# jennyzhang0215/DGL-KGAT

Hardware: AMD Instinct MI355X
Metric: propagation-layer edges/sec on amazon-book CKG; achieved HBM GB/s vs peak (higher is better)
Workload: dtype f32; 1 GPU; amazon-book-shaped CKG N=159251 E=3663302 R=41, 3 layers, embed_dim=64, fp32; partition=none, setup_steps=1, full=False

## Files before the change

### dgl-kgat_amd/_lib.py

```python
import ctypes as C
import hashlib
import os
import subprocess

_HERE = os.path.dirname(os.path.abspath(__file__))
CSRC = os.path.join(_HERE, "csrc")
SO_PATH = os.path.join(_HERE, "libkgat_hip.so")
SOURCES = {
    "kgat_graph.hip": [],
    "kgat_permute.hip": [],
    "kgat_spmm.hip": [],
    "kgat_spmm_max.hip": [],
    "kgat_spmm_kmax.hip": [],
    "kgat_spmm_bi.hip": ["-mllvm", "-amdgpu-mfma-vgpr-form=1"],
    "kgat_softmax.hip": [],
    "kgat_att.hip": [],
    "kgat_att_persistent.hip": ["-mllvm", "-amdgpu-mfma-vgpr-form=1"],
    "kgat_dense.hip": ["-mllvm", "-amdgpu-mfma-vgpr-form=1"],
    "kgat_transr.hip": [],
    "kgat_transr_rank.hip": ["-mllvm", "-amdgpu-mfma-vgpr-form=1"],
    "kgat_eval.hip": [],
    "kgat_eval_topk.hip": ["-mllvm", "-amdgpu-mfma-vgpr-form=1"],
    "kgat_optim.hip": [],
    "kgat_bpr.hip": [],
# ... 69 lines not shown
    "kgat_transr_loss_grad_f32": (_i32, [_i64, _i32, _i32, _i32, _i64, _p, _p, _p, _p, _p, _p, _p, C.c_float, _p, _p,
                                         _p, _p, _p, _sz, _p]),
    "kgat_transr_forward_f32": (_i32, [_i64, _i32, _i32, _i32, _i64, _p, _p, _p, _p, _p, _p, _p, C.c_float, _p, _p, _sz, _p]),
    "kgat_transr_backward_f32": (_i32, [_i64, _i32, _i32, _i32, _i64, _p, _p, _p, _p, _p, _p, _p, _p, _p, _sz, _p]),
    "kgat_bi_interaction_f32": (_i32, [_i64, _i32, _i32, _p, _p, C.c_float, _p, _p, _i64, _p]),
    "kgat_spmm_tile_edges": (_i32, [_i64, _i32]),
    "kgat_l2_normalize_rows_f32": (_i32, [_i64, _i32, _p, _p, _i64, _p]),
    "kgat_readout_concat_f32": (_i32, [_i64, _i32, _p, _p, _p, _p, _i64, _p]),
    "kgat_sddmm_dot_f32": (_i32, [_i64, _i32, _p, _p, _p, _p, _p, _p]),
    "kgat_gather_probe_f32": (_i32, [_i64, _i32, _p, _p, _p, _p]),
    "kgat_gather_f32": (_i32, [_i64, _p, _p, _p, _p]),
    "kgat_gather_i32": (_i32, [_i64, _p, _p, _p, _p]),
    "kgat_permute_tile": (_i32, []),
    "kgat_permute_supported": (_i32, [_i64]),
    "kgat_permute_f32": (_i32, [_i64, _p, _p, _p, _p, _p, _p, _p]),
    "kgat_eval_supported": (_i32, [_i32, _i32]),
    "kgat_eval_items_elems": (_i64, [_i64, _i32]),
    "kgat_eval_items_kmajor_f32": (_i32, [_i64, _i32, _p, _i64, _p, _p, _p]),
    "kgat_eval_workspace_bytes": (_sz, [_i64, _i64, _i32, _i32]),
    "kgat_bpr_workspace_bytes": (_sz, [_i64, _i32]),
    "kgat_bpr_loss_f32": (_i32, [_i64, _i32, _p, _i64, _i64, _p, _p, _p, C.c_float, _p, _p, _p, _sz, _p]),
    "kgat_bpr_grad_f32": (_i32, [_i64, _i32, _p, _i64, _i64, _p, _p, _p, _p, C.c_float, _p, _p, _p, _sz, _p]),
    "kgat_transr_sorted_bytes": (_sz, [_i64, _i32]),
    "kgat_transr_presort_f32": (_i32, [_i64, _i32, _i64, _i64, _p, _p, _p, _p, _p, _sz, _p]),
    "kgat_transr_step_workspace_bytes": (_sz, [_i64, _i32, _i32, _i32]),
    "kgat_transr_adam_step_f32": (_i32, [_i64, _i32, _i32, _i32, _i64, _p, _p, _p, _p, _p, _p, _p, _p, _p, _p, _p,
                                         C.c_double, C.c_double, C.c_double, C.c_double, C.c_float, _p, _p, C.c_uint64,
                                         _p, _sz, _p]),
    "kgat_adam_max_tensors": (_i32, []),
    "kgat_adam_step_f32": (_i32, [_i32, _p, _p, _p, _p, _p, _p, C.c_double, C.c_double, C.c_double, C.c_double, _i32, _p]),
# ... 200 lines not shown
```

### dgl-kgat_amd/csrc/kgat_permute.hip

```cpp
#include "kgat_common.h"

#ifndef KGAT_PERMUTE_TILE
#define KGAT_PERMUTE_TILE 16384
#endif

namespace {

using namespace kgat;

constexpr int kPermTile = KGAT_PERMUTE_TILE;
constexpr int kPermThreads = 1024;
constexpr int kPermMinRun = 16;
static_assert(kPermTile % (kPermThreads * 8) == 0 && kPermTile <= 65536, "tile: whole 8-item rounds, 16-bit slots");

typedef uint32_t u32x4 __attribute__((ext_vector_type(4)));

__device__ __forceinline__ void scatter_to_lds(const uint32_t* __restrict__ val, const uint16_t* __restrict__ slot, int cnt,
                                               uint32_t* lds) {
  constexpr int kRounds = kPermTile / (kPermThreads * 8);
  u32x4 lo[kRounds], hi[kRounds], s[kRounds];
#pragma unroll
  for (int r = 0; r < kRounds; ++r) {
    const int i = (r * kPermThreads + (int)threadIdx.x) * 8;
    if (i + 8 <= cnt) {
// ... 44 lines not shown
  __shared__ __attribute__((aligned(16))) uint32_t lds[kPermTile];
  constexpr int kRounds = kPermTile / (kPermThreads * 4);
  const int64_t base = (int64_t)blockIdx.x * kPermTile;
  const int cnt = (int)(n - base < kPermTile ? n - base : kPermTile);
  scatter_to_lds(tmp + base, slot_b + base, cnt, lds);
  __syncthreads();
#pragma unroll
  for (int r = 0; r < kRounds; ++r) {
    const int i = (r * kPermThreads + (int)threadIdx.x) * 4;
    if (i + 4 <= cnt) {
      __builtin_nontemporal_store(*reinterpret_cast<const u32x4*>(lds + i), reinterpret_cast<u32x4*>(out + base + i));
    } else {
      for (int k = i; k < cnt; ++k) out[base + k] = lds[k];
    }
  }
}

}

extern "C" {

int kgat_permute_tile(void) { return kPermTile; }

int kgat_permute_supported(int64_t n) {
  return n >= 0 && n * kPermMinRun <= (int64_t)kPermTile * kPermTile ? 1 : 0;
}

int kgat_permute_f32(int64_t n, const uint16_t* slot_a, const int32_t* dst_a, const uint16_t* slot_b, const float* in,
                     float* out, float* tmp, kgat_stream_t stream) {
  KGAT_CHECK_ARG(n >= 0, "permute: negative size");
// ... 23 lines not shown
```

### dgl-kgat_amd/csrc/kgat_softmax.hip

```cpp
#include <math.h>

#include "kgat_common.h"

#define SM_LD_LOGIT(p) (*(p))
#define SM_LD_MAP(p) __builtin_nontemporal_load(p)
namespace kgat {

constexpr float kFixScale = 1099511627776.0f;
constexpr float kFixInv = 1.0f / 1099511627776.0f;

__global__ void softmax_init_kernel(int64_t n, float* __restrict__ M,
                                    unsigned long long* __restrict__ Z) {
  const int64_t i = (int64_t)blockIdx.x * blockDim.x + threadIdx.x;
  if (i < n) {
    M[i] = -INFINITY;
    Z[i] = 0ull;
  }
}

__device__ __forceinline__ void atomic_max_f32(float* addr, float v) {
  if (v == 0.f) v = 0.f;
  if (v >= 0.f) atomicMax(reinterpret_cast<int*>(addr), __float_as_int(v));
  else atomicMin(reinterpret_cast<unsigned int*>(addr), __float_as_uint(v));
}
// ... 99 lines not shown
    e[k] = valid ? (eid ? eid[p[k]] : (int32_t)p[k]) : 0;
  }
#pragma unroll
  for (int k = 0; k < kItems; ++k) {
    s[k] = r[k] >= 0 ? (IN_CSR ? logits[p[k]] : logits[e[k]]) : 0.f;
    m[k] = r[k] >= 0 ? M[r[k]] : 0.f;
    z[k] = r[k] >= 0 ? Z[r[k]] : 1ull;
  }
#pragma unroll
  for (int k = 0; k < kItems; ++k) {
    if (r[k] < 0) continue;
    const float a = expf(s[k] - m[k]) / ((float)z[k] * kFixInv);
    if (out_csr) out_csr[p[k]] = a;
    if (out) out[e[k]] = a;
  }
}

constexpr int kSmMaxEPL = 16;
constexpr int64_t kSmSmallEdges = 8 << 20;
template <int EPL> struct SmGeom {
  static constexpr int EPW = kWave * EPL;
};
constexpr float kSmNegBig = -3.0e38f;

struct __attribute__((aligned(16))) SmCarry {
  int32_t row;
  int32_t count;
  float m, s;
  int32_t head;
  int32_t last;
  int32_t pad0, pad1;
};

__device__ __forceinline__ float sm_exp(float x) {
  x = fmaxf(x, -128.0f);
  const float t = x * 1.44269504088896341f;
  const float lo = fmaf(x, 1.44269504088896341f, -t) + x * 1.92596299112661746e-8f;
  return __builtin_amdgcn_exp2f(t) * fmaf(lo, 0.693147180559945309f, 1.0f);
}

__device__ __forceinline__ void sm_combine(float& m, float& s, float m2, float s2) {
  const bool keep = m >= m2;
  const float e = sm_exp(keep ? m2 - m : m - m2);
  const float big = keep ? s : s2, small = keep ? s2 : s;
  s = fmaf(small, e, big);
  m = keep ? m : m2;
}

__device__ __forceinline__ int64_t sm_wave_index() {
  return (int64_t)blockIdx.x * (256 / kWave) + __builtin_amdgcn_readfirstlane((int)(threadIdx.x / kWave));
}

template <int CTRL, int ROW_MASK>
__device__ __forceinline__ float sm_dpp(float old, float src) {
  return __int_as_float(__builtin_amdgcn_update_dpp(__float_as_int(old), __float_as_int(src), CTRL, ROW_MASK, 0xf, false));
}
template <int CTRL>
__device__ __forceinline__ int32_t sm_dpp_i(int32_t old, int32_t src) {
  return __builtin_amdgcn_update_dpp(old, src, CTRL, 0xf, 0xf, false);
}

// ... 226 lines not shown

template <bool IN_CSR, int kSmEPL>
__global__ __launch_bounds__(256) void softmax_local_kernel(
    int64_t e0, int64_t e1, int aligned, const int32_t* __restrict__ indptr, const int32_t* __restrict__ row_of,
    const int32_t* __restrict__ eid, const float* __restrict__ logits, float* __restrict__ out,
    float* __restrict__ out_csr, SmCarry* __restrict__ carry) {
  constexpr int kSmEPW = SmGeom<kSmEPL>::EPW;
  const int64_t w = sm_wave_index();
  const int64_t base = e0 + w * kSmEPW;
  if (base >= e1) return;
  const int64_t end = base + kSmEPW < e1 ? base + kSmEPW : e1;
  if (aligned && end - base == kSmEPW)
    sm_sweep<IN_CSR, kSmEPL, true>(e0, e1, w, base, end, indptr, row_of, eid, logits, out, out_csr, carry);
  else
    sm_sweep<IN_CSR, kSmEPL, false>(e0, e1, w, base, end, indptr, row_of, eid, logits, out, out_csr, carry);
}

__device__ __forceinline__ void sm_chain_total(const SmCarry* __restrict__ carry, int32_t head, int32_t last,
                                               int lane, float& M, float& S) {
  const SmCarry h = carry[2 * (int64_t)head + 1];
  float m = h.m, s = h.s;
  for (int64_t j0 = (int64_t)head + 1; j0 <= last; j0 += kWave) {
    const int64_t j = j0 + lane;
    float pm = kSmNegBig, ps = 0.f;
    if (j <= last) {
      const SmCarry f = carry[2 * j];
      pm = f.m; ps = f.s;
    }
#pragma unroll
    for (int d = 1; d < kWave; d <<= 1) {
      const float m2 = __shfl_down(pm, d, kWave), s2 = __shfl_down(ps, d, kWave);
      if ((lane & (2 * d - 1)) == 0) sm_combine(pm, ps, m2, s2);
    }
    pm = __shfl(pm, 0, kWave); ps = __shfl(ps, 0, kWave);
    sm_combine(m, s, pm, ps);
  }
  M = m; S = s;
}

__device__ __forceinline__ void sm_rescale_span(int64_t lo, int64_t hi, int lane, float f,
                                                const int32_t* __restrict__ eid, float* __restrict__ out,
                                                float* __restrict__ out_csr) {
  constexpr int U = 8;
  for (int64_t p0 = lo; p0 < hi; p0 += U * kWave) {
    int64_t e[U];
    float x[U];
#pragma unroll
    for (int u = 0; u < U; ++u) {
      const int64_t p = p0 + u * kWave + lane;
      const int64_t pc = p < hi ? p : hi - 1;
      e[u] = out ? (int64_t)eid[pc] : pc;
    }
// ... 86 lines not shown
#pragma unroll
  for (int off = kWave / 2; off > 0; off >>= 1) acc += __shfl_xor(acc, off, kWave);
  for (int32_t p = beg + lane; p < end; p += kWave) {
    const int32_t e = HAS_EID ? eid[p] : p;
    gs[e] = a[e] * g[e] - a[e] * acc;
  }
}

}

using namespace kgat;

template <bool IN_CSR, int EPL>
static void launch_softmax_sweep(int64_t e_begin, int64_t e_end, const int32_t* indptr, const int32_t* row_of,
                                 const int32_t* eid, const float* logits, float* out, float* out_csr, SmCarry* carry,
                                 hipStream_t st) {
  const int64_t n_waves = (e_end - e_begin + SmGeom<EPL>::EPW - 1) / SmGeom<EPL>::EPW;
  const unsigned blocks = (unsigned)((n_waves + 3) / 4);
  const uintptr_t bits = (uintptr_t)row_of | (uintptr_t)eid | (uintptr_t)out_csr | (IN_CSR ? (uintptr_t)logits : 0);
  const int aligned = (bits % 16 == 0 && e_begin % 4 == 0) ? 1 : 0;
  hipLaunchKernelGGL((softmax_local_kernel<IN_CSR, EPL>), dim3(blocks), dim3(256), 0, st, e_begin, e_end, aligned, indptr,
                     row_of, eid, logits, out, out_csr, carry);
  hipLaunchKernelGGL((softmax_cut_rows_kernel<EPL>), dim3(blocks), dim3(256), 0, st, e_begin, e_end, eid, out, out_csr,
                     (const SmCarry*)carry);
}

extern "C" {

size_t kgat_edge_softmax_workspace_bytes(int64_t n_nodes, int64_t n_edges) {
  (void)n_nodes;
  constexpr int kMinEPW = SmGeom<8>::EPW;
  const size_t n_waves = (size_t)((n_edges > 0 ? n_edges : 0) + kMinEPW - 1) / kMinEPW;
  return align_up((2 * n_waves + 2) * sizeof(SmCarry), 256);
}

int kgat_edge_softmax_f32(int64_t n_nodes, int64_t e_begin, int64_t e_end, const int32_t* indptr,
                          const int32_t* row_of, const int32_t* eid, const float* logits,
// ... 11 lines not shown
    set_error("edge_softmax: workspace too small");
    return KGAT_E_WORKSPACE;
  }
  hipStream_t st = as_stream(stream);
  SmCarry* carry = static_cast<SmCarry*>(workspace);
  const bool small = ne < kSmSmallEdges;
  if (logits_in_csr_order) {
    if (small) launch_softmax_sweep<true, 8>(e_begin, e_end, indptr, row_of, eid, logits, out, out_csr, carry, st);
    else launch_softmax_sweep<true, 16>(e_begin, e_end, indptr, row_of, eid, logits, out, out_csr, carry, st);
  } else {
    if (small) launch_softmax_sweep<false, 8>(e_begin, e_end, indptr, row_of, eid, logits, out, out_csr, carry, st);
    else launch_softmax_sweep<false, 16>(e_begin, e_end, indptr, row_of, eid, logits, out, out_csr, carry, st);
  }
  KGAT_CHECK_LAUNCH("edge_softmax");
  return KGAT_OK;
}

size_t kgat_edge_softmax_3pass_workspace_bytes(int64_t n_nodes) {
  const size_t n = (size_t)(n_nodes > 0 ? n_nodes : 1);
  return align_up(n * sizeof(float), 256) + align_up(n * sizeof(unsigned long long), 256);
}

int kgat_edge_softmax_3pass_f32(int64_t n_nodes, int64_t e_begin, int64_t e_end,
                                const int32_t* row_of, const int32_t* eid, const float* logits,
                                int logits_in_csr_order, float* out, float* out_csr, void* workspace,
                                size_t workspace_bytes, kgat_stream_t stream) {
  KGAT_CHECK_ARG(n_nodes >= 0 && e_begin >= 0 && e_end >= e_begin && e_end < INT32_MAX,
                 "edge_softmax_3pass: bad size");
  if (e_end == e_begin) return KGAT_OK;
  KGAT_CHECK_ARG(row_of && logits && workspace, "edge_softmax_3pass: null pointer");
// ... 56 lines not shown
```

### dgl-kgat_amd/graph.py

```python
from collections import namedtuple
from collections.abc import MutableMapping

import os

import numpy as np
import torch

from . import ops
from .options import options
from .function import BuiltinMessage, BuiltinReduce
from .lazy import LazyEdgeWeights, pending_csr_weights

ALL = "__ALL__"


class DGLError(Exception):
    """Same role as dgl.DGLError: misuse of the graph API."""


def _as_id_array(x, name):
    if isinstance(x, torch.Tensor):
        x = x.detach().cpu().numpy()
    x = np.asarray(x)
    if x.ndim == 0:
# ... 174 lines not shown
            et32 = etype.to(device=dev, dtype=torch.int32).contiguous()
            rel_ptr, idx = ops.group_by_relation(ops.gather(csr.eid, et32), int(n_rel))
            dst_g = ops.gather(idx, csr.row_of)
            gid, gptr, g_node, n_groups = ops.head_groups(rel_ptr, dst_g)
            hit = ((etype._version, int(n_rel)),
                   RelGroups(rel_ptr, ops.gather(idx, csr.eid), ops.gather(idx, csr.col), dst_g, idx,
                             gid, gptr, g_node, n_groups, {}), etype)
            c["rel_groups"] = hit
        return hit[1]

    def permuted(self, name, src_of, values, out=None):
        planned = (values.dtype == torch.float32 and ops.permute_supported(src_of.numel())
                   and values.data_ptr() % 16 == 0 and (out is None or out.data_ptr() % 16 == 0))
        if not planned:
            return ops.gather(src_of, values, out=out)
        c = self._cache(values.device)
        plan = c.get(("permute_plan", name))
        if plan is None or plan[0] is not src_of:
            plan = c[("permute_plan", name)] = (src_of, ops.permute_plan(src_of))
        tmp = c.get("permute_tmp")
        if tmp is None or tmp.numel() != src_of.numel():
            tmp = c["permute_tmp"] = torch.empty(src_of.numel(), dtype=torch.float32, device=values.device)
        return ops.permute(plan[1], values, out=out, tmp=tmp)

    def weight_in_csr_order(self, w_flat):
        c = self._cache(w_flat.device)
        key = (w_flat.data_ptr(), w_flat._version, w_flat.numel())
        hit = c.get("w_csr")
        if hit is None or hit[0] != key:
            hit = (key, self.permuted("csr_eid", self.csr(w_flat.device).eid, w_flat), w_flat)
            c["w_csr"] = hit
        return hit[1]

    def weight_in_rev_order(self, w_flat):
        c = self._cache(w_flat.device)
        key = (w_flat.data_ptr(), w_flat._version, w_flat.numel())
        hit = c.get("w_rev")
        if hit is None or hit[0] != key:
# ... 432 lines not shown
                                 ent_c, W_c, rel_c, pos_g=groups.pos_g, algo=one_algo)[1]

        forms = {"fused": (fused, "grouped"), "folded": (lambda: two_launch(True), "csr"),
                 "split": (lambda: two_launch(False), "csr"), "one": (one, "csr")}
        form, one_algo = options.att_form if algo == "auto" else algo, "auto"
        if form in ("auto", "race"):
            race_run = (lambda f: forms[f][0]()) if form == "race" else None
            form = groups.g_tab.get(("form", d, k))
            if form is None:
                form = groups.g_tab[("form", d, k)] = self._pick_attention_form(groups, n_rel, d, k, race_run)
        elif form not in forms:
            form, one_algo = "one", form
        run, order = forms[form]
        logits = run()
        st.last_att_form = (form, groups.n_groups)
        _, a_csr = ops.edge_softmax(csr.indptr, csr.row_of, _gpos_csr(groups) if order == "grouped" else csr.eid, logits,
                                    in_csr_order=order == "csr", want_out=False, want_csr=True)
        from . import lazy as lazy_mod
        if lazy is None:
            lazy = lazy_mod.enabled()
        elif lazy:
            lazy_mod._guard_legacy_to_dlpack()
        a = torch.empty((st.n_edges, 1), dtype=torch.float32, device=dev)
        a_flat = a.view(-1)

        def fill():
            st.permuted("csr_pos", st.csr_pos(dev), a_csr, out=a_flat)
            st.remember_weight(a_flat, a_csr)
        if not lazy:
            fill()
            return a
        return LazyEdgeWeights(a, fill, st, a_csr)
```

### dgl-kgat_amd/ops.py

```python
from collections import namedtuple

import torch

from . import _lib
from ._lib import KGATLibraryError, check

SPMM_MUL_SELF = 1
SPMM_DEFER_FINISH = 2
SPMM_ALGO = {"auto": 0, "merge": 1, "rows": 2, "generic": 3, "merge1": 4}
ATT_ALGO = {"auto": 0, "mfma": 1, "generic": 2, "mfma_chunk": 3}


def _stream(t):
    return torch.cuda.current_stream(t.device).cuda_stream


class KernelTimer:
    active = None

    def __init__(self):
        self.records = []

    def __enter__(self):
        KernelTimer.active = self
# ... 516 lines not shown
    out_csr = torch.empty_like(logits) if want_csr else None
    with _timed("edge_softmax", (e1 - e0,)):
        if three_pass:
            ws = _workspace(lib.kgat_edge_softmax_3pass_workspace_bytes(n_nodes), logits.device)
            check(lib.kgat_edge_softmax_3pass_f32(n_nodes, e0, e1, _ptr(row_of), _ptr(eid), _ptr(logits),
                                                  1 if in_csr_order else 0, _ptr(out), _ptr(out_csr), _ptr(ws),
                                                  ws.numel(), _stream(logits)), "kgat_edge_softmax_3pass_f32")
        else:
            ws = _workspace(lib.kgat_edge_softmax_workspace_bytes(n_nodes, e1 - e0), logits.device)
            check(lib.kgat_edge_softmax_f32(n_nodes, e0, e1, _ptr(indptr), _ptr(row_of), _ptr(eid), _ptr(logits),
                                            1 if in_csr_order else 0, _ptr(out), _ptr(out_csr), _ptr(ws),
                                            ws.numel(), _stream(logits)), "kgat_edge_softmax_f32")
    return out, out_csr


def edge_softmax_bwd(indptr, eid, a, grad_a, row_range=None):
    a = _need(a, torch.float32, "a")
    grad_a = _need(grad_a, torch.float32, "grad_a", a.shape)
    indptr = _need(indptr, torch.int32, "indptr")
    if eid is not None:
        eid = _need(eid, torch.int32, "eid", a.shape)
    row0, n_rows = (0, indptr.numel() - 1) if row_range is None else row_range
    out = torch.zeros_like(a)
    if a.numel() == 0:
        return out
    check(_lib.load().kgat_edge_softmax_bwd_f32(n_rows, row0, _ptr(indptr), _ptr(eid), _ptr(a),
                                                _ptr(grad_a), _ptr(out), _stream(a)),
          "kgat_edge_softmax_bwd_f32")
    return out

# ... 582 lines not shown
def sddmm_dot(src, dst, X, G):
    X = _need(X, torch.float32, "X")
    G = _need(G, torch.float32, "grad_out")
    src = _need(src, torch.int32, "src")
    dst = _need(dst, torch.int32, "dst", src.shape)
    if X.shape[1] != G.shape[1]:
        raise ValueError("feature widths differ")
    out = torch.empty(src.numel(), dtype=torch.float32, device=X.device)
    check(_lib.load().kgat_sddmm_dot_f32(src.numel(), X.shape[1], _ptr(src), _ptr(dst), _ptr(X), _ptr(G),
                                         _ptr(out), _stream(X)), "kgat_sddmm_dot_f32")
    return out


__all__ = ["csr_from_coo", "group_by_relation", "invert_permutation", "row_order_by_degree", "gather",
           "permute_tile", "permute_supported", "permute_plan_arrays", "permute_plan", "permute", "PermutePlan",
           "att_score", "att_score_split", "att_score_split_supported", "att_score_folded_supported", "att_score_fused", "att_pack_records", "att_score_fused_supported", "fold_tiles", "fold_tile_cost", "bi_interaction_train", "add3_rows", "bi_interaction_bwd_pre", "bi_interaction_bwd_input", "bi_interaction_bwd_input_supported", "bi_interaction_bwd_weight", "sum_partials", "mul2", "dropout_keep_mask", "transr_loss_grad", "transr_supported", "transr_presort", "transr_adam_step", "TransRAdamState", "head_groups", "edge_softmax", "edge_softmax_bwd", "spmm", "spmm_workspace", "sddmm_dot",
           "bi_interaction", "bi_interaction_supported", "l2_normalize_rows", "readout_concat",
           "FORMS", "aggregator", "aggregator_supported", "aggregator_bwd_supported", "aggregator_train",
           "aggregator_bwd_input", "aggregator_bwd_weight",
           "KGATLibraryError"]


def eval_supported(F, K):
    return bool(_lib.load().kgat_eval_supported(int(F), int(K)))


def eval_recall_ndcg(emb, user_ids, item_ids, train_ptr, train_items, test_ptr, test_items, K, want_topk=False):
    if emb.dtype != torch.float32 or not emb.is_cuda or emb.dim() != 2 or emb.stride(1) != 1:
        raise KGATLibraryError("eval_recall_ndcg: `emb` must be a float32 HIP matrix with unit column stride")
    F, stride = emb.shape[1], emb.stride(0)
    user_ids = _need(user_ids, torch.int32, "user_ids")
# ... 304 lines not shown
```

### dgl-kgat_amd/options.py

```python
import contextlib
import os


def _flag(name, default):
    v = os.environ.get(name)
    return default if v is None else v not in ("", "0")


class Options:
    __slots__ = ("att_f32_products", "att_form", "fold_tile_cost", "fuse_bi", "gnn_defer_finish", "lazy_edge_weights",
                 "eager_edge_weights", "partition_row_weight", "force_collectives", "exchange", "exchange_chunks")

    def __init__(self):
        self.load()

    def load(self):
        e = os.environ
        self.att_f32_products = _flag("KGAT_ATT_F32_PRODUCTS", False)
        self.att_form = e.get("KGAT_ATT_FORM", "auto")
        cost = e.get("KGAT_FOLD_TILE_COST")
        self.fold_tile_cost = tuple(int(x) for x in cost.split(",")) if cost else None
        self.fuse_bi = _flag("KGAT_FUSE_BI", False)
        self.gnn_defer_finish = _flag("KGAT_GNN_DEFER_FINISH", True)
        self.lazy_edge_weights = _flag("KGAT_LAZY_EDGE_WEIGHTS", False)
        self.eager_edge_weights = bool(e.get("KGAT_EAGER_EDGE_WEIGHTS"))
        rw = e.get("KGAT_PARTITION_ROW_WEIGHT")
        self.partition_row_weight = int(rw) if rw else None
        self.force_collectives = _flag("KGAT_FORCE_COLLECTIVES", False)
        self.exchange = e.get("KGAT_EXCHANGE", "allreduce")
        self.exchange_chunks = int(e.get("KGAT_EXCHANGE_CHUNKS", "1"))


options = Options()


def reload():
    options.load()
    return options


# ... 11 lines not shown
```

### include/kgat_hip.h

```cpp
#ifndef KGAT_HIP_H_
#define KGAT_HIP_H_

#include <stddef.h>
#include <stdint.h>

#ifdef __cplusplus
extern "C" {
#endif

#define KGAT_ABI_VERSION 16

enum {
  KGAT_OK = 0,
  KGAT_E_BADARG = -1,
  KGAT_E_UNSUPPORTED = -2,
  KGAT_E_WORKSPACE = -3,
  KGAT_E_HIP = -4
};

enum {
  KGAT_SPMM_MUL_SELF = 1,
  KGAT_SPMM_DEFER_FINISH = 2
};

// ... 182 lines not shown
                               kgat_stream_t stream);

int kgat_readout_concat_f32(int64_t n_rows, int n_blocks, const float* const* blocks, const int* widths,
                            const int* normalize, float* out, int64_t out_stride, kgat_stream_t stream);

int kgat_gather_f32(int64_t n, const int32_t* index, const float* in, float* out,
                    kgat_stream_t stream);
int kgat_gather_i32(int64_t n, const int32_t* index, const int32_t* in, int32_t* out,
                    kgat_stream_t stream);

int kgat_permute_tile(void);
int kgat_permute_supported(int64_t n);
int kgat_permute_f32(int64_t n, const uint16_t* slot_a, const int32_t* dst_a, const uint16_t* slot_b, const float* in,
                     float* out, float* tmp, kgat_stream_t stream);

int kgat_add3_rows_f32(int64_t n_rows, int d, const float* a, int64_t a_stride, const float* b, const float* c, float* out,
                       kgat_stream_t stream);
int kgat_bi_interaction_bwd_pre_f32(int64_t n_rows, int d_out, const float* h_out, const float* grad_a,
                                    const float* grad_b, const float* grad_norm, int64_t grad_norm_stride,
                                    float negative_slope, float drop_p, uint64_t seed, int64_t row0, float* grad_z,
                                    kgat_stream_t stream);
int kgat_bi_interaction_bwd_input_supported(int d_in, int d_out);
int64_t kgat_bi_interaction_bwd_weight_partials(int64_t n_rows);
int kgat_sum_partials_f32(int n_sets, const float* const* partials_host, float* const* out_host,
                          const int64_t* n_partials_host, const int64_t* n_elems_host, kgat_stream_t stream);
int kgat_mul2_f32(int64_t n, const float* a, const float* b, const float* c, float* ab, float* ac,
                  kgat_stream_t stream);

int kgat_spmm_tile_edges(int64_t n_edges, int D);
int kgat_aggregator_supported(int form, int d_in, int d_out);
// ... 159 lines not shown
```

Baseline: 25.27 billion edges/s.

## Fuse edge-softmax cut-row fixup into the permute bin kernel

Adds an edge-softmax path that skips the separate cut-rows rescale kernel and instead applies the cross-range row normalization inside the first pass of the two-pass permute. The CSR-ordered weights are fixed up in registers while they are being scattered to LDS, so one full read/write pass over the edge weights goes away. It is enabled by default when not in lazy mode and sizes fit. The cost is a heavier permute kernel that does carry-chain walks and extra carry loads, with more register pressure.

```diff
diff --git a/dgl-kgat_amd/_lib.py b/dgl-kgat_amd/_lib.py
--- a/dgl-kgat_amd/_lib.py
+++ b/dgl-kgat_amd/_lib.py
@@ -107,6 +107,8 @@
     "kgat_permute_tile": (_i32, []),
     "kgat_permute_supported": (_i32, [_i64]),
     "kgat_permute_f32": (_i32, [_i64, _p, _p, _p, _p, _p, _p, _p]),
+    "kgat_edge_softmax_permuted_supported": (_i32, [_i64, _i64]),
+    "kgat_edge_softmax_permuted_f32": (_i32, [_i64, _i64, _i64, _p, _p, _p, _p, _i32, _p, _p, _p, _p, _p, _p, _p, _sz, _p]),
     "kgat_eval_supported": (_i32, [_i32, _i32]),
     "kgat_eval_items_elems": (_i64, [_i64, _i32]),
     "kgat_eval_items_kmajor_f32": (_i32, [_i64, _i32, _p, _i64, _p, _p, _p]),
diff --git a/dgl-kgat_amd/csrc/kgat_permute.hip b/dgl-kgat_amd/csrc/kgat_permute.hip
--- a/dgl-kgat_amd/csrc/kgat_permute.hip
+++ b/dgl-kgat_amd/csrc/kgat_permute.hip
@@ -1,4 +1,5 @@
 #include "kgat_common.h"
+#include "kgat_softmax_carry.h"
 
 #ifndef KGAT_PERMUTE_TILE
 #define KGAT_PERMUTE_TILE 16384
@@ -82,6 +83,209 @@
       for (int k = i; k < cnt; ++k) out[base + k] = lds[k];
     }
   }
+}
+
+struct PermCut {
+  int32_t row;
+  int32_t count;
+  int32_t head, last;
+  bool walk;
+  float m;
+  float M, S;
+};
+
+__device__ __forceinline__ PermCut perm_cut_a(const SmCarry& ca, const SmCarry& pv, int64_t g, int32_t top) {
+  PermCut c;
+  c.row = ca.row; c.count = ca.count; c.m = ca.m; c.walk = false;
+  c.head = ca.head < 0 ? 0 : (ca.head < top ? ca.head : top);
+  c.last = ca.last < 0 ? 0 : (ca.last < top ? ca.last : top);
+  c.M = pv.m; c.S = pv.s;
+  if (ca.row >= 0) {
+    if (ca.head == g - 1 && ca.last == g) sm_combine(c.M, c.S, ca.m, ca.s);
+    else c.walk = true;
+  }
+  return c;
+}
+
+__device__ __forceinline__ PermCut perm_cut_b(const SmCarry& cb, const SmCarry& nx, int64_t g, int32_t top) {
+  PermCut c;
+  c.row = cb.row; c.count = cb.count; c.m = cb.m; c.walk = false;
+  c.head = cb.head < 0 ? 0 : (cb.head < top ? cb.head : top);
+  c.last = cb.last < 0 ? 0 : (cb.last < top ? cb.last : top);
+  c.M = cb.m; c.S = cb.s;
+  if (cb.row >= 0) {
+    if (cb.last == g + 1) sm_combine(c.M, c.S, nx.m, nx.s);
+    else c.walk = true;
+  }
+  return c;
+}
+
+template <int kCuts>
+__device__ __forceinline__ void perm_walk_chains(const SmCarry* __restrict__ carry, PermCut (&c)[kCuts],
+                                                 const int (&own)[kCuts], const int (&src)[kCuts], float* walk_m,
+                                                 float* walk_s, int lane) {
+#pragma unroll 1
+  for (int e = 0; e < kCuts; ++e) {
+    int32_t head = 0, last = 0;
+    int slot = -1;
+#pragma unroll
+    for (int k = 0; k < kCuts; ++k)
+      if (k == e) { head = c[k].head; last = c[k].last; slot = c[k].walk ? own[k] : -1; }
+    if (slot < 0) continue;
+    int32_t hv = head;
+    asm volatile("" : "+v"(hv));
+    const SmCarry* hp = carry + (2 * (int64_t)hv + 1);
+    float M = hp->m, S = hp->s;
+    float pm[4], ps[4];
+    const int64_t j0 = (int64_t)head + 1;
+#pragma unroll
+    for (int b = 0; b < 4; ++b) sm_chain_load(carry, j0 + b * kWave, last, lane, pm[b], ps[b]);
+    sm_chain_trees<4>(pm, ps, lane);
+#pragma unroll
+    for (int b = 0; b < 4; ++b)
+      if (j0 + b * kWave <= last) sm_combine(M, S, pm[b], ps[b]);
+    sm_chain_rest<4>(carry, j0 + 4 * kWave, last, lane, M, S);
+    if (lane == 0) { walk_m[slot] = M; walk_s[slot] = S; }
+#pragma unroll
+    for (int k = 0; k < kCuts; ++k)
+      if (k == e) { c[k].M = M; c[k].S = S; }
+  }
+  __syncthreads();
+#pragma unroll
+  for (int k = 0; k < kCuts; ++k)
+    if (c[k].walk && own[k] < 0) { c[k].M = walk_m[src[k]]; c[k].S = walk_s[src[k]]; }
+}
+
+__device__ __forceinline__ uint32_t perm_scaled(uint32_t bits, float f) { return __float_as_uint(__uint_as_float(bits) * f); }
+
+template <int EPW>
+__global__ __launch_bounds__(kPermThreads) void permute_bin_softmax_kernel(int64_t n, const uint16_t* __restrict__ slot_a,
+                                                                           const int32_t* __restrict__ dst_a,
+                                                                           const SmCarry* __restrict__ carry, uint32_t* w,
+                                                                           uint32_t* __restrict__ tmp) {
+  static_assert(EPW % (kWave * 8) == 0, "a wavefront round (8 x 64 positions) lies inside one range");
+  __shared__ __attribute__((aligned(16))) uint32_t lds[kPermTile];
+  constexpr int kPer = kPermTile / kPermThreads;
+  constexpr int kRounds = kPermTile / (kPermThreads * 8);
+  const int64_t base = (int64_t)blockIdx.x * kPermTile;
+  const int cnt = (int)(n - base < kPermTile ? n - base : kPermTile);
+  const int lane = (int)threadIdx.x % kWave;
+  const int wave = __builtin_amdgcn_readfirstlane((int)threadIdx.x / kWave);
+  const int64_t n_ranges = (n + EPW - 1) / EPW;
+  constexpr int kRanges = kPermTile / EPW;
+  static_assert((kRanges & (kRanges - 1)) == 0, "ranges per chunk: a power of two (slot masks)");
+  __shared__ float walk_m[2 * kRanges], walk_s[2 * kRanges];
+  uint32_t dst[kPer];
+#pragma unroll
+  for (int j = 0; j < kPer; ++j) {
+    const int i = j * kPermThreads + (int)threadIdx.x;
+    dst[j] = i < cnt ? (uint32_t)__builtin_nontemporal_load(dst_a + base + i) : 0xffffffffu;
+  }
+  uint32_t* val = w + base;
+  const uint16_t* slot = slot_a + base;
+  u32x4 lo[kRounds], hi[kRounds], s[kRounds];
+#pragma unroll
+  for (int r = 0; r < kRounds; ++r) {
+    const int i = (r * kPermThreads + (int)threadIdx.x) * 8;
+    if (i + 8 <= cnt) {
+      lo[r] = *reinterpret_cast<const u32x4*>(val + i);
+      hi[r] = *reinterpret_cast<const u32x4*>(val + i + 4);
+      s[r] = __builtin_nontemporal_load(reinterpret_cast<const u32x4*>(slot + i));
+    }
+  }
+  SmCarry ca[kRounds], cb[kRounds], pv[kRounds], nx[kRounds];
+  int64_t g[kRounds];
+  bool live[kRounds];
+#pragma unroll
+  for (int r = 0; r < kRounds; ++r) {
+    const int64_t gr = (base + (int64_t)(r * kPermThreads + wave * kWave) * 8) / EPW;
+    live[r] = gr < n_ranges;
+    g[r] = live[r] ? gr : n_ranges - 1;
+    ca[r] = carry[2 * g[r]];
+    cb[r] = carry[2 * g[r] + 1];
+    pv[r] = carry[2 * (g[r] > 0 ? g[r] - 1 : 0) + 1];
+    nx[r] = carry[2 * (g[r] + 1 < n_ranges ? g[r] + 1 : g[r])];
+  }
+  const int32_t top = (int32_t)(n_ranges - 1);
+  const int64_t g_first = base / EPW;
+  PermCut cut[2 * kRounds];
+  int own[2 * kRounds], src[2 * kRounds];
+#pragma unroll
+  for (int r = 0; r < kRounds; ++r) {
+    cut[2 * r] = perm_cut_a(ca[r], pv[r], g[r], top);
+    cut[2 * r + 1] = perm_cut_b(cb[r], nx[r], g[r], top);
+    if (!live[r]) cut[2 * r].walk = cut[2 * r + 1].walk = false;
+    const int gl = (int)(g[r] - g_first) & (kRanges - 1);
+    const int64_t hl = cut[2 * r].head - g_first;
+    own[2 * r] = gl == 0 ? 0 : -1;
+    src[2 * r] = hl < 0 ? 0 : (2 * (int)hl + 1) & (2 * kRanges - 1);
+    own[2 * r + 1] = src[2 * r + 1] = 2 * gl + 1;
+  }
+  perm_walk_chains(carry, cut, own, src, walk_m, walk_s, lane);
+#pragma unroll
+  for (int r = 0; r < kRounds; ++r) {
+    const int i = (r * kPermThreads + (int)threadIdx.x) * 8;
+    const int q0 = (int)((base + i) % EPW);
+    const PermCut &a = cut[2 * r], &b = cut[2 * r + 1];
+    const int len = (int)(n - g[r] * EPW < EPW ? n - g[r] * EPW : EPW);
+    const int na = a.row >= 0 ? a.count : 0, b0 = b.row >= 0 ? len - b.count : EPW;
+    const float fa = a.row >= 0 ? sm_exp(a.m - a.M) / a.S : 1.0f, fb = b.row >= 0 ? sm_exp(b.m - b.M) / b.S : 1.0f;
+    if (i + 8 <= cnt) {
+      if (q0 < na || q0 + 7 >= b0) {
+#pragma unroll
+        for (int k = 0; k < 4; ++k) {
+          lo[r][k] = q0 + k < na ? perm_scaled(lo[r][k], fa) : (q0 + k >= b0 ? perm_scaled(lo[r][k], fb) : lo[r][k]);
+          hi[r][k] = q0 + 4 + k < na ? perm_scaled(hi[r][k], fa) : (q0 + 4 + k >= b0 ? perm_scaled(hi[r][k], fb) : hi[r][k]);
+        }
+        if (q0 < na || q0 + 3 >= b0) *reinterpret_cast<u32x4*>(val + i) = lo[r];
+        if (q0 + 4 < na || q0 + 7 >= b0) *reinterpret_cast<u32x4*>(val + i + 4) = hi[r];
+      }
+#pragma unroll
+      for (int k = 0; k < 4; ++k) {
+        lds[(s[r][k >> 1] >> (16 * (k & 1))) & (kPermTile - 1)] = lo[r][k];
+        lds[(s[r][2 + (k >> 1)] >> (16 * (k & 1))) & (kPermTile - 1)] = hi[r][k];
+      }
+    } else {
+      for (int k = i; k < cnt; ++k) {
+        const int q = q0 + (k - i);
+        uint32_t v = val[k];
+        if (q < na || q >= b0) {
+          v = perm_scaled(v, q < na ? fa : fb);
+          val[k] = v;
+        }
+        lds[slot[k] & (kPermTile - 1)] = v;
+      }
+    }
+  }
+  __syncthreads();
+#pragma unroll
+  for (int j = 0; j < kPer; ++j)
+    if (dst[j] < (uint64_t)n) tmp[dst[j]] = lds[j * kPermThreads + (int)threadIdx.x];
+}
+
+}
+
+namespace kgat {
+
+bool permute_softmax_fits(int epw) { return epw > 0 && kPermTile % epw == 0 && epw % (kWave * 8) == 0; }
+
+int permute_softmax_launch(int epw, int64_t n, const uint16_t* slot_a, const int32_t* dst_a, const uint16_t* slot_b,
+                           const SmCarry* carry, float* w, float* out, float* tmp, hipStream_t st) {
+  const dim3 grid((unsigned)((n + kPermTile - 1) / kPermTile)), block(kPermThreads);
+  uint32_t* wv = reinterpret_cast<uint32_t*>(w);
+  uint32_t* tv = reinterpret_cast<uint32_t*>(tmp);
+  if (epw == SmGeom<8>::EPW && permute_softmax_fits(epw))
+    hipLaunchKernelGGL(permute_bin_softmax_kernel<SmGeom<8>::EPW>, grid, block, 0, st, n, slot_a, dst_a, carry, wv, tv);
+  else if (epw == SmGeom<16>::EPW && permute_softmax_fits(epw))
+    hipLaunchKernelGGL(permute_bin_softmax_kernel<SmGeom<16>::EPW>, grid, block, 0, st, n, slot_a, dst_a, carry, wv, tv);
+  else {
+    set_error("permute_softmax: ranges of %d positions do not tile chunks of %d", epw, kPermTile);
+    return KGAT_E_UNSUPPORTED;
+  }
+  KGAT_CHECK_LAUNCH("permute_bin_softmax");
+  hipLaunchKernelGGL(permute_place_kernel, grid, block, 0, st, n, slot_b, (const uint32_t*)tv, reinterpret_cast<uint32_t*>(out));
+  KGAT_CHECK_LAUNCH("permute_place");
+  return KGAT_OK;
 }
 
 }
diff --git a/dgl-kgat_amd/csrc/kgat_softmax.hip b/dgl-kgat_amd/csrc/kgat_softmax.hip
--- a/dgl-kgat_amd/csrc/kgat_softmax.hip
+++ b/dgl-kgat_amd/csrc/kgat_softmax.hip
@@ -1,6 +1,7 @@
 #include <math.h>
 
 #include "kgat_common.h"
+#include "kgat_softmax_carry.h"
 
 #define SM_LD_LOGIT(p) (*(p))
 #define SM_LD_MAP(p) __builtin_nontemporal_load(p)
@@ -137,37 +138,6 @@
     if (out_csr) out_csr[p[k]] = a;
     if (out) out[e[k]] = a;
   }
-}
-
-constexpr int kSmMaxEPL = 16;
-constexpr int64_t kSmSmallEdges = 8 << 20;
-template <int EPL> struct SmGeom {
-  static constexpr int EPW = kWave * EPL;
-};
-constexpr float kSmNegBig = -3.0e38f;
-
-struct __attribute__((aligned(16))) SmCarry {
-  int32_t row;
-  int32_t count;
-  float m, s;
-  int32_t head;
-  int32_t last;
-  int32_t pad0, pad1;
-};
-
-__device__ __forceinline__ float sm_exp(float x) {
-  x = fmaxf(x, -128.0f);
-  const float t = x * 1.44269504088896341f;
-  const float lo = fmaf(x, 1.44269504088896341f, -t) + x * 1.92596299112661746e-8f;
-  return __builtin_amdgcn_exp2f(t) * fmaf(lo, 0.693147180559945309f, 1.0f);
-}
-
-__device__ __forceinline__ void sm_combine(float& m, float& s, float m2, float s2) {
-  const bool keep = m >= m2;
-  const float e = sm_exp(keep ? m2 - m : m - m2);
-  const float big = keep ? s : s2, small = keep ? s2 : s;
-  s = fmaf(small, e, big);
-  m = keep ? m : m2;
 }
 
 __device__ __forceinline__ int64_t sm_wave_index() {
@@ -424,28 +394,6 @@
     sm_sweep<IN_CSR, kSmEPL, true>(e0, e1, w, base, end, indptr, row_of, eid, logits, out, out_csr, carry);
   else
     sm_sweep<IN_CSR, kSmEPL, false>(e0, e1, w, base, end, indptr, row_of, eid, logits, out, out_csr, carry);
-}
-
-__device__ __forceinline__ void sm_chain_total(const SmCarry* __restrict__ carry, int32_t head, int32_t last,
-                                               int lane, float& M, float& S) {
-  const SmCarry h = carry[2 * (int64_t)head + 1];
-  float m = h.m, s = h.s;
-  for (int64_t j0 = (int64_t)head + 1; j0 <= last; j0 += kWave) {
-    const int64_t j = j0 + lane;
-    float pm = kSmNegBig, ps = 0.f;
-    if (j <= last) {
-      const SmCarry f = carry[2 * j];
-      pm = f.m; ps = f.s;
-    }
-#pragma unroll
-    for (int d = 1; d < kWave; d <<= 1) {
-      const float m2 = __shfl_down(pm, d, kWave), s2 = __shfl_down(ps, d, kWave);
-      if ((lane & (2 * d - 1)) == 0) sm_combine(pm, ps, m2, s2);
-    }
-    pm = __shfl(pm, 0, kWave); ps = __shfl(ps, 0, kWave);
-    sm_combine(m, s, pm, ps);
-  }
-  M = m; S = s;
 }
 
 __device__ __forceinline__ void sm_rescale_span(int64_t lo, int64_t hi, int lane, float f,
@@ -562,13 +510,14 @@
 template <bool IN_CSR, int EPL>
 static void launch_softmax_sweep(int64_t e_begin, int64_t e_end, const int32_t* indptr, const int32_t* row_of,
                                  const int32_t* eid, const float* logits, float* out, float* out_csr, SmCarry* carry,
-                                 hipStream_t st) {
+                                 hipStream_t st, bool cut_rows = true) {
   const int64_t n_waves = (e_end - e_begin + SmGeom<EPL>::EPW - 1) / SmGeom<EPL>::EPW;
   const unsigned blocks = (unsigned)((n_waves + 3) / 4);
   const uintptr_t bits = (uintptr_t)row_of | (uintptr_t)eid | (uintptr_t)out_csr | (IN_CSR ? (uintptr_t)logits : 0);
   const int aligned = (bits % 16 == 0 && e_begin % 4 == 0) ? 1 : 0;
   hipLaunchKernelGGL((softmax_local_kernel<IN_CSR, EPL>), dim3(blocks), dim3(256), 0, st, e_begin, e_end, aligned, indptr,
                      row_of, eid, logits, out, out_csr, carry);
+  if (!cut_rows) return;
   hipLaunchKernelGGL((softmax_cut_rows_kernel<EPL>), dim3(blocks), dim3(256), 0, st, e_begin, e_end, eid, out, out_csr,
                      (const SmCarry*)carry);
 }
@@ -610,6 +559,54 @@
   }
   KGAT_CHECK_LAUNCH("edge_softmax");
   return KGAT_OK;
+}
+
+int kgat_edge_softmax_permuted_supported(int64_t e_begin, int64_t e_end) {
+  if (e_begin != 0 || e_end < 0 || e_end >= INT32_MAX || !kgat_permute_supported(e_end)) return 0;
+  return permute_softmax_fits(e_end < kSmSmallEdges ? SmGeom<8>::EPW : SmGeom<16>::EPW) ? 1 : 0;
+}
+
+int kgat_edge_softmax_permuted_f32(int64_t n_nodes, int64_t e_begin, int64_t e_end, const int32_t* indptr,
+                                   const int32_t* row_of, const int32_t* eid, const float* logits,
+                                   int logits_in_csr_order, const uint16_t* slot_a, const int32_t* dst_a,
+                                   const uint16_t* slot_b, float* out, float* out_csr, float* tmp, void* workspace,
+                                   size_t workspace_bytes, kgat_stream_t stream) {
+  KGAT_CHECK_ARG(n_nodes >= 0 && e_begin >= 0 && e_end >= e_begin && e_end < INT32_MAX,
+                 "edge_softmax_permuted: bad size");
+  if (!kgat_edge_softmax_permuted_supported(e_begin, e_end)) {
+    set_error("edge_softmax_permuted: needs e_begin = 0 (got %lld) and a size kgat_permute_supported takes (got %lld): "
+              "use kgat_edge_softmax_f32 and kgat_permute_f32 / kgat_gather_f32", (long long)e_begin, (long long)e_end);
+    return KGAT_E_UNSUPPORTED;
+  }
+  if (e_end == 0) return KGAT_OK;
+  KGAT_CHECK_ARG(indptr && row_of && logits && workspace, "edge_softmax_permuted: null pointer");
+  KGAT_CHECK_ARG(slot_a && dst_a && slot_b && out && out_csr && tmp, "edge_softmax_permuted: null pointer");
+  KGAT_CHECK_ARG(eid != nullptr || logits_in_csr_order, "edge_softmax_permuted: edge-id ordered input needs eid");
+  KGAT_CHECK_ARG(out != out_csr && out != tmp && out_csr != tmp && (const float*)out_csr != logits &&
+                     (const float*)out != logits && (const float*)tmp != logits,
+                 "edge_softmax_permuted: logits, out, out_csr and tmp must be four buffers");
+  if (!(aligned16(slot_a) && aligned16(slot_b) && aligned16(out) && aligned16(out_csr) && aligned16(tmp) &&
+        aligned16(workspace))) {
+    set_error("edge_softmax_permuted: slot_a, slot_b, out, out_csr, tmp and workspace must be 16-byte aligned");
+    return KGAT_E_UNSUPPORTED;
+  }
+  if (workspace_bytes < kgat_edge_softmax_workspace_bytes(n_nodes, e_end)) {
+    set_error("edge_softmax_permuted: workspace too small");
+    return KGAT_E_WORKSPACE;
+  }
+  hipStream_t st = as_stream(stream);
+  SmCarry* carry = static_cast<SmCarry*>(workspace);
+  const bool small = e_end < kSmSmallEdges;
+  if (logits_in_csr_order) {
+    if (small) launch_softmax_sweep<true, 8>(0, e_end, indptr, row_of, eid, logits, nullptr, out_csr, carry, st, false);
+    else launch_softmax_sweep<true, 16>(0, e_end, indptr, row_of, eid, logits, nullptr, out_csr, carry, st, false);
+  } else {
+    if (small) launch_softmax_sweep<false, 8>(0, e_end, indptr, row_of, eid, logits, nullptr, out_csr, carry, st, false);
+    else launch_softmax_sweep<false, 16>(0, e_end, indptr, row_of, eid, logits, nullptr, out_csr, carry, st, false);
+  }
+  KGAT_CHECK_LAUNCH("edge_softmax_permuted: sweep");
+  return permute_softmax_launch(small ? SmGeom<8>::EPW : SmGeom<16>::EPW, e_end, slot_a, dst_a, slot_b, carry, out_csr, out,
+                                tmp, st);
 }
 
 size_t kgat_edge_softmax_3pass_workspace_bytes(int64_t n_nodes) {
diff --git a/dgl-kgat_amd/csrc/kgat_softmax_carry.h b/dgl-kgat_amd/csrc/kgat_softmax_carry.h
--- /dev/null
+++ b/dgl-kgat_amd/csrc/kgat_softmax_carry.h
@@ -0,0 +1,97 @@
+#pragma once
+#include "kgat_common.h"
+
+namespace kgat {
+
+constexpr int kSmMaxEPL = 16;
+constexpr int64_t kSmSmallEdges = 8 << 20;
+template <int EPL> struct SmGeom {
+  static constexpr int EPW = kWave * EPL;
+};
+constexpr float kSmNegBig = -3.0e38f;
+
+struct __attribute__((aligned(16))) SmCarry {
+  int32_t row;
+  int32_t count;
+  float m, s;
+  int32_t head;
+  int32_t last;
+  int32_t pad0, pad1;
+};
+
+__device__ __forceinline__ float sm_exp(float x) {
+  x = fmaxf(x, -128.0f);
+  const float t = x * 1.44269504088896341f;
+  const float lo = fmaf(x, 1.44269504088896341f, -t) + x * 1.92596299112661746e-8f;
+  return __builtin_amdgcn_exp2f(t) * fmaf(lo, 0.693147180559945309f, 1.0f);
+}
+
+__device__ __forceinline__ void sm_combine(float& m, float& s, float m2, float s2) {
+  const bool keep = m >= m2;
+  const float e = sm_exp(keep ? m2 - m : m - m2);
+  const float big = keep ? s : s2, small = keep ? s2 : s;
+  s = fmaf(small, e, big);
+  m = keep ? m : m2;
+}
+
+template <int kB>
+__device__ __forceinline__ void sm_chain_trees(float (&pm)[kB], float (&ps)[kB], int lane) {
+#pragma unroll
+  for (int d = 1; d < kWave; d <<= 1) {
+    float m2[kB], s2[kB];
+#pragma unroll
+    for (int b = 0; b < kB; ++b) { m2[b] = __shfl_down(pm[b], d, kWave); s2[b] = __shfl_down(ps[b], d, kWave); }
+    if ((lane & (2 * d - 1)) == 0) {
+#pragma unroll
+      for (int b = 0; b < kB; ++b) sm_combine(pm[b], ps[b], m2[b], s2[b]);
+    }
+  }
+#pragma unroll
+  for (int b = 0; b < kB; ++b) { pm[b] = __shfl(pm[b], 0, kWave); ps[b] = __shfl(ps[b], 0, kWave); }
+}
+
+__device__ __forceinline__ void sm_chain_total(const SmCarry* __restrict__ carry, int32_t head, int32_t last,
+                                               int lane, float& M, float& S) {
+  const SmCarry h = carry[2 * (int64_t)head + 1];
+  float m = h.m, s = h.s;
+  for (int64_t j0 = (int64_t)head + 1; j0 <= last; j0 += kWave) {
+    const int64_t j = j0 + lane;
+    float pm[1] = {kSmNegBig}, ps[1] = {0.f};
+    if (j <= last) {
+      const SmCarry f = carry[2 * j];
+      pm[0] = f.m; ps[0] = f.s;
+    }
+    sm_chain_trees<1>(pm, ps, lane);
+    sm_combine(m, s, pm[0], ps[0]);
+  }
+  M = m; S = s;
+}
+
+__device__ __forceinline__ void sm_chain_load(const SmCarry* __restrict__ carry, int64_t j0, int32_t last, int lane,
+                                              float& pm, float& ps) {
+  const int64_t j = j0 + lane;
+  const SmCarry* f = carry + 2 * (j <= last ? j : (int64_t)last);
+  const float fm = f->m, fs = f->s;
+  pm = j <= last ? fm : kSmNegBig;
+  ps = j <= last ? fs : 0.f;
+}
+
+template <int kAhead>
+__device__ __forceinline__ void sm_chain_rest(const SmCarry* __restrict__ carry, int64_t j0, int32_t last, int lane,
+                                              float& m, float& s) {
+  for (; j0 <= last; j0 += kAhead * kWave) {
+    float pm[kAhead], ps[kAhead];
+#pragma unroll
+    for (int b = 0; b < kAhead; ++b) sm_chain_load(carry, j0 + b * kWave, last, lane, pm[b], ps[b]);
+    sm_chain_trees<kAhead>(pm, ps, lane);
+#pragma unroll
+    for (int b = 0; b < kAhead; ++b)
+      if (j0 + b * kWave <= last) sm_combine(m, s, pm[b], ps[b]);
+  }
+}
+
+bool permute_softmax_fits(int epw);
+int permute_softmax_launch(int epw, int64_t n, const uint16_t* slot_a, const int32_t* dst_a, const uint16_t* slot_b,
+                           const SmCarry* carry, float* w, float* out, float* tmp, hipStream_t st);
+
+}
diff --git a/dgl-kgat_amd/graph.py b/dgl-kgat_amd/graph.py
--- a/dgl-kgat_amd/graph.py
+++ b/dgl-kgat_amd/graph.py
@@ -212,14 +212,18 @@
                    and values.data_ptr() % 16 == 0 and (out is None or out.data_ptr() % 16 == 0))
         if not planned:
             return ops.gather(src_of, values, out=out)
-        c = self._cache(values.device)
+        plan, tmp = self.permute_plan(name, src_of, values.device)
+        return ops.permute(plan, values, out=out, tmp=tmp)
+
+    def permute_plan(self, name, src_of, device):
+        c = self._cache(device)
         plan = c.get(("permute_plan", name))
         if plan is None or plan[0] is not src_of:
             plan = c[("permute_plan", name)] = (src_of, ops.permute_plan(src_of))
         tmp = c.get("permute_tmp")
         if tmp is None or tmp.numel() != src_of.numel():
-            tmp = c["permute_tmp"] = torch.empty(src_of.numel(), dtype=torch.float32, device=values.device)
-        return ops.permute(plan[1], values, out=out, tmp=tmp)
+            tmp = c["permute_tmp"] = torch.empty(src_of.numel(), dtype=torch.float32, device=device)
+        return plan[1], tmp
 
     def weight_in_csr_order(self, w_flat):
         c = self._cache(w_flat.device)
@@ -682,8 +686,6 @@
         run, order = forms[form]
         logits = run()
         st.last_att_form = (form, groups.n_groups)
-        _, a_csr = ops.edge_softmax(csr.indptr, csr.row_of, _gpos_csr(groups) if order == "grouped" else csr.eid, logits,
-                                    in_csr_order=order == "csr", want_out=False, want_csr=True)
         from . import lazy as lazy_mod
         if lazy is None:
             lazy = lazy_mod.enabled()
@@ -691,6 +693,16 @@
             lazy_mod._guard_legacy_to_dlpack()
         a = torch.empty((st.n_edges, 1), dtype=torch.float32, device=dev)
         a_flat = a.view(-1)
+        index = _gpos_csr(groups) if order == "grouped" else csr.eid
+        if (not lazy and options.softmax_permuted and logits.numel() and ops.edge_softmax_permuted_supported(logits.numel())
+                and a_flat.data_ptr() % 16 == 0):
+            plan, tmp = st.permute_plan("csr_pos", st.csr_pos(dev), dev)
+            _, a_csr = ops.edge_softmax_permuted(csr.indptr, csr.row_of, index, logits, plan, in_csr_order=order == "csr",
+                                                 out=a_flat, tmp=tmp)
+            st.remember_weight(a_flat, a_csr)
+            return a
+        _, a_csr = ops.edge_softmax(csr.indptr, csr.row_of, index, logits, in_csr_order=order == "csr", want_out=False,
+                                    want_csr=True)
 
         def fill():
             st.permuted("csr_pos", st.csr_pos(dev), a_csr, out=a_flat)
diff --git a/dgl-kgat_amd/ops.py b/dgl-kgat_amd/ops.py
--- a/dgl-kgat_amd/ops.py
+++ b/dgl-kgat_amd/ops.py
@@ -554,6 +554,29 @@
     return out, out_csr
 
 
+def edge_softmax_permuted_supported(n_edges, e_begin=0):
+    return bool(_lib.load().kgat_edge_softmax_permuted_supported(int(e_begin), int(e_begin) + int(n_edges)))
+
+
+def edge_softmax_permuted(indptr, row_of, eid, logits, plan, in_csr_order=False, out=None, tmp=None):
+    logits = _need(logits, torch.float32, "logits", (plan.n,))
+    indptr = _need(indptr, torch.int32, "indptr")
+    row_of = _need(row_of, torch.int32, "row_of", logits.shape)
+    eid = _need(eid, torch.int32, "eid", logits.shape)
+    out = torch.empty_like(logits) if out is None else _need(out, torch.float32, "out", (plan.n,))
+    tmp = torch.empty_like(logits) if tmp is None else _need(tmp, torch.float32, "tmp", (plan.n,))
+    out_csr = torch.empty_like(logits)
+    n_nodes = indptr.numel() - 1
+    lib = _lib.load()
+    with _timed("edge_softmax_permuted", (plan.n,)):
+        ws = _workspace(lib.kgat_edge_softmax_workspace_bytes(n_nodes, plan.n), logits.device)
+        check(lib.kgat_edge_softmax_permuted_f32(n_nodes, 0, plan.n, _ptr(indptr), _ptr(row_of), _ptr(eid), _ptr(logits),
+                                                 1 if in_csr_order else 0, _ptr(plan.slot_a), _ptr(plan.dst_a),
+                                                 _ptr(plan.slot_b), _ptr(out), _ptr(out_csr), _ptr(tmp), _ptr(ws),
+                                                 ws.numel(), _stream(logits)), "kgat_edge_softmax_permuted_f32")
+    return out, out_csr
+
+
 def edge_softmax_bwd(indptr, eid, a, grad_a, row_range=None):
     a = _need(a, torch.float32, "a")
     grad_a = _need(grad_a, torch.float32, "grad_a", a.shape)
@@ -1166,7 +1189,7 @@
 
 __all__ = ["csr_from_coo", "group_by_relation", "invert_permutation", "row_order_by_degree", "gather",
            "permute_tile", "permute_supported", "permute_plan_arrays", "permute_plan", "permute", "PermutePlan",
-           "att_score", "att_score_split", "att_score_split_supported", "att_score_folded_supported", "att_score_fused", "att_pack_records", "att_score_fused_supported", "fold_tiles", "fold_tile_cost", "bi_interaction_train", "add3_rows", "bi_interaction_bwd_pre", "bi_interaction_bwd_input", "bi_interaction_bwd_input_supported", "bi_interaction_bwd_weight", "sum_partials", "mul2", "dropout_keep_mask", "transr_loss_grad", "transr_supported", "transr_presort", "transr_adam_step", "TransRAdamState", "head_groups", "edge_softmax", "edge_softmax_bwd", "spmm", "spmm_workspace", "sddmm_dot",
+           "att_score", "att_score_split", "att_score_split_supported", "att_score_folded_supported", "att_score_fused", "att_pack_records", "att_score_fused_supported", "fold_tiles", "fold_tile_cost", "bi_interaction_train", "add3_rows", "bi_interaction_bwd_pre", "bi_interaction_bwd_input", "bi_interaction_bwd_input_supported", "bi_interaction_bwd_weight", "sum_partials", "mul2", "dropout_keep_mask", "transr_loss_grad", "transr_supported", "transr_presort", "transr_adam_step", "TransRAdamState", "head_groups", "edge_softmax", "edge_softmax_permuted", "edge_softmax_permuted_supported", "edge_softmax_bwd", "spmm", "spmm_workspace", "sddmm_dot",
            "bi_interaction", "bi_interaction_supported", "l2_normalize_rows", "readout_concat",
            "FORMS", "aggregator", "aggregator_supported", "aggregator_bwd_supported", "aggregator_train",
            "aggregator_bwd_input", "aggregator_bwd_weight",
diff --git a/dgl-kgat_amd/options.py b/dgl-kgat_amd/options.py
--- a/dgl-kgat_amd/options.py
+++ b/dgl-kgat_amd/options.py
@@ -9,7 +9,7 @@
 
 class Options:
     __slots__ = ("att_f32_products", "att_form", "fold_tile_cost", "fuse_bi", "gnn_defer_finish", "lazy_edge_weights",
-                 "eager_edge_weights", "partition_row_weight", "force_collectives", "exchange", "exchange_chunks")
+                 "eager_edge_weights", "softmax_permuted", "partition_row_weight", "force_collectives", "exchange", "exchange_chunks")
 
     def __init__(self):
         self.load()
@@ -24,6 +24,7 @@
         self.gnn_defer_finish = _flag("KGAT_GNN_DEFER_FINISH", True)
         self.lazy_edge_weights = _flag("KGAT_LAZY_EDGE_WEIGHTS", False)
         self.eager_edge_weights = bool(e.get("KGAT_EAGER_EDGE_WEIGHTS"))
+        self.softmax_permuted = _flag("KGAT_SOFTMAX_PERMUTED", True)
         rw = e.get("KGAT_PARTITION_ROW_WEIGHT")
         self.partition_row_weight = int(rw) if rw else None
         self.force_collectives = _flag("KGAT_FORCE_COLLECTIVES", False)
diff --git a/include/kgat_hip.h b/include/kgat_hip.h
--- a/include/kgat_hip.h
+++ b/include/kgat_hip.h
@@ -220,6 +220,13 @@
 int kgat_permute_f32(int64_t n, const uint16_t* slot_a, const int32_t* dst_a, const uint16_t* slot_b, const float* in,
                      float* out, float* tmp, kgat_stream_t stream);
 
+int kgat_edge_softmax_permuted_supported(int64_t e_begin, int64_t e_end);
+int kgat_edge_softmax_permuted_f32(int64_t n_nodes, int64_t e_begin, int64_t e_end, const int32_t* indptr,
+                                   const int32_t* row_of, const int32_t* eid, const float* logits,
+                                   int logits_in_csr_order, const uint16_t* slot_a, const int32_t* dst_a,
+                                   const uint16_t* slot_b, float* out, float* out_csr, float* tmp, void* workspace,
+                                   size_t workspace_bytes, kgat_stream_t stream);
+
 int kgat_add3_rows_f32(int64_t n_rows, int d, const float* a, int64_t a_stride, const float* b, const float* c, float* out,
                        kgat_stream_t stream);
 int kgat_bi_interaction_bwd_pre_f32(int64_t n_rows, int d_out, const float* h_out, const float* grad_a,
```

New measurement: 25.73 billion edges/s (median of 6 runs). +1.8%, better.
